# dune-community/pylrbms

Hardware: AMD Instinct MI355X
Metric: offline project+estimate throughput (higher is better)
Workload: dtype f64; 1 GPU; BASELINE.json config 3: 2D multiscale diffusion, 32x32 subdomains, k_c=4 (n=384 DG DoFs, n_rt=208 RT0 DoFs per subdomain), Q=2, local basis dim 40; subdomains=1024, N=40, Q=2, parallelism=subdomain tiles x1

## Files before the change

include/lrbms_hip.h:

```cpp
#ifndef LRBMS_HIP_H
#define LRBMS_HIP_H

#include <stdint.h>

#ifdef __cplusplus
extern "C" {
#endif

#define LRBMS_OK 0
#define LRBMS_E_INVALID (-1)
#define LRBMS_E_HIP (-2)
#define LRBMS_E_STATE (-3)
#define LRBMS_E_NOT_CONVERGED (-4)

#define LRBMS_NS 16

typedef struct lrbms_ctx lrbms_ctx;

typedef struct {
  int32_t kx, ky, n_T, n_rt, n_vertices, ncf;
  double hx, hy;
  double kappa[4];
  const int32_t* nb_elem;
  const int32_t* nb_face;
// ... 95 lines not shown
void* lrbms_ctx_aux_stream(lrbms_ctx* ctx, int32_t i);

#define LRBMS_OPT_OSWALD_VERTEX_PATCH 9
#define LRBMS_OPT_OSWALD_ZERO_ON_SUBDOMAIN_BOUNDARY 1
#define LRBMS_OPT_ACCUMULATE_COUPLING_ACROSS_Q 2
#define LRBMS_OPT_STREAMS 3
#define LRBMS_OPT_F1_KSPLIT 4
#define LRBMS_OPT_F1_FORM 5
#define LRBMS_OPT_COARSE 6
#define LRBMS_OPT_SOLVE_VALU 7
#define LRBMS_OPT_ESTIMATE_VALU 8
#define LRBMS_OPT_PREP_LDS 10
#define LRBMS_OPT_F2_FORM 11
#define LRBMS_OPT_SIDE_TABLES 12
#define LRBMS_OPT_THIN_MERGE 13
int lrbms_ctx_set_option(lrbms_ctx* ctx, int32_t option, int32_t value);

int lrbms_set_diagonal_neighbours(lrbms_ctx* ctx, const int32_t* nbr_diag);

int lrbms_fused_set_subset(lrbms_ctx* ctx, const int32_t* subset, int32_t count);

int lrbms_kernel_timing(lrbms_ctx* ctx, int32_t enable);
int lrbms_kernel_timing_read(lrbms_ctx* ctx, char* names, int64_t names_cap, double* ms, int32_t cap, int32_t* count);

int lrbms_project_estimate_fused_phase(lrbms_ctx* ctx, int32_t phase, int32_t Q, int32_t N, const double* V, const double* F,
                                       const double* A_diag, const double* A_cpl, const double* P_diag, const double* b,
                                       const double* ebar, const double* caa, const double* Aab, const double* Bbb, double* work,
                                       double* B_sys, double* rhs_red, double* E_red, double* M_red, double* G_nc, double* r_fd,
                                       double* G_rdd, double* G_bb, double* G_ab, double* G_aa, void* stream);

// ... 132 lines not shown
```

pylrbms_amd/_isa_check.py:

```python
import re


class IsaCheckError(RuntimeError):
    pass


def _functions(path):
    cur, out = None, {}
    with open(path) as fh:
        for ln in fh:
            m = re.match(r'^(_Z\w+):\s+; @', ln)
            if m:
                cur = m.group(1)
                out[cur] = []
                continue
            if cur is not None:
                if ln.startswith('.Lfunc_end'):
                    cur = None
                    continue
                out[cur].append(ln.rstrip('\n'))
    return out


def _metadata(path):
# ... 9 lines not shown
                continue
            m = re.match(r'^\s+(?:- )?\.(private_segment_fixed_size|sgpr_spill_count|vgpr_spill_count|vgpr_count|agpr_count):\s+(\d+)', ln)
            if m:
                key, val = m.group(1), int(m.group(2))
                if cur is not None and key not in out[cur]:
                    out[cur][key] = val
                else:
                    pending[key] = val
            if re.match(r'^\s+- \.', ln) and cur is not None and '.name' not in ln:
                cur = None
                m2 = re.match(r'^\s+- \.(\w+):\s+(\d+)', ln)
                pending = {m2.group(1): int(m2.group(2))} if m2 else {}
    return out


def _producer_loops(lines):
    in_asm, tags = False, []
    for ln in lines:
        s = ln.strip()
        if s.startswith(';;#ASMSTART'):
            in_asm = True
        tags.append(in_asm)
        if s.startswith(';;#ASMEND'):
            in_asm = False
    starts = [i for i, ln in enumerate(lines) if re.match(r'^(\.LBB\d+_\d+:|; %bb\.\d+:)', ln)]
    starts.append(len(lines))
    loops = {}
    for k in range(len(starts) - 1):
        head = lines[starts[k]]
        m = re.match(r'^\.LBB\d+_(\d+):.*Loop Header', head)
        owner = m.group(1) if m else None
        if owner is None:
            m = re.search(r'in Loop: Header=BB\d+_(\d+)', head)
            owner = m.group(1) if m else None
        if owner is not None:
            loops.setdefault(owner, []).extend(range(starts[k], starts[k + 1]))
    out = [idx for idx in loops.values() if any(tags[i] and 'global_load' in lines[i] for i in idx)]
    return out, tags


def _regs(tok):
    m = re.fullmatch(r'v(\d+)', tok)
    if m:
        return {int(m.group(1))}
    m = re.fullmatch(r'v\[(\d+):(\d+)\]', tok)
    if m:
        return set(range(int(m.group(1)), int(m.group(2)) + 1))
    return set()


def _operands(line):
    body = line.split(';')[0].strip()
# ... 120 lines not shown
        raise IsaCheckError('thin-kernel register check failed:\n  ' + '\n  '.join(problems))
    return sorted(report)


def check_fused_isa(asm_path):
    fns = _functions(asm_path)
    meta = _metadata(asm_path)
    report, problems = [], []
    with open(asm_path) as fh:
        try:
            report += check_thin_registers(fh.read())
        except IsaCheckError as exc:
            problems.append(str(exc))
    seen = 0
    for name, lines in fns.items():
        m = re.search(r'\dk_f(1u|1v|1|2g|2)I((?:Li\d+E)+)E', name) or re.search(r'\dk_f(1w)()E4Tmpl', name)
        if not m:
            continue
        kernel = 'k_f{}<{}>'.format(m.group(1), ','.join(re.findall(r'Li(\d+)E', m.group(2))))
        md = meta.get(name, {})
        spills = md.get('vgpr_spill_count', 0)
        scratch_lines = [i for i, ln in enumerate(lines) if re.match(r'\s+scratch_', ln)]
        in_asm = False
        first_asm_load = None
        for i, ln in enumerate(lines):
            st = ln.strip()
            if st.startswith(';;#ASMSTART'):
                in_asm = True
            elif st.startswith(';;#ASMEND'):
                in_asm = False
            elif in_asm and 'global_load' in ln:
                first_asm_load = i
                break
        wide = m.group(1) in ('1', '1u') and re.findall(r'Li(\d+)E', m.group(2))[0] == '4'
        if (spills or scratch_lines or md.get('private_segment_fixed_size', 0)) and not wide:
            problems.append('{}: scratch {} bytes, {} spilled VGPRs'.format(kernel, md.get('private_segment_fixed_size'), spills))
        if spills > 8:
            problems.append('{}: {} spilled VGPRs'.format(kernel, spills))
        if scratch_lines and first_asm_load is not None and max(scratch_lines) >= first_asm_load:
            problems.append('{}: scratch instruction behind the first asm-managed load (line {} >= {})'.format(
                kernel, max(scratch_lines), first_asm_load))
        lean = m.group(1) in ('1v', '1w')
        uses_asm_prefetch = any(';;#ASMSTART' in ln for ln in lines) and \
            any('global_load' in ln for ln in lines if True) and \
            any(re.search(r'^\s+s_waitcnt vmcnt\((?!0\))\d+\)\s*$' if not lean else r'^\s+s_waitcnt vmcnt\(0\)\s*$', ln) for ln in lines)
        loops, tags = _producer_loops(lines)
        if m.group(1) == '1' and kernel.endswith(',0>'):
            report.append('{}: compiler-managed loads, VGPRs {}'.format(kernel, md.get('vgpr_count')))
            continue
        if not loops or not uses_asm_prefetch:
            problems.append('{}: no producer loop with asm-managed prefetch found'.format(kernel))
            continue
        seen += 1
        if lean:
            loop_blocks = set()
            starts_all = sorted({0} | {i for i, ln in enumerate(lines) if re.match(r'^\.LBB\d+_\d+:', ln)})
            for idx in loops:
                members = set(idx)
                loop_blocks |= {b for b in starts_all if b in members}
            hz = _inflight_register_hazards(lines, tags, region=None, prologue_of=loop_blocks)
            if hz:
                problems.append('{}: compiler-emitted instruction touches the destination of an asm load of the PROLOGUE still in flight: {}'.format(
                    kernel, hz[:3]))
        for idx in loops:
            hazards = _inflight_register_hazards(lines, tags, region=idx)
            if hazards:
                problems.append('{}: compiler-emitted instruction touches the destination of an asm load still in flight: {}'.format(
                    kernel, hazards[:3]))
            a, b = idx[0], idx[-1]
            asm_waits = sorted({lines[k].strip() for k in idx if tags[k] and 'vmcnt' in lines[k]})
            counts = [int(x) for w in asm_waits for x in re.findall(r'vmcnt\((\d+)\)', w)]
            own_waits = [lines[k].strip() for k in idx if not tags[k] and re.search(r's_waitcnt.*vmcnt', lines[k])]
            own_vmem = [lines[k].strip() for k in idx
                        if not tags[k] and re.match(r'\s+(global_|buffer_|scratch_|flat_)', lines[k])]
            if not counts or (min(counts) == 0 and not lean):
                problems.append('{}: producer loop waits {} (expected one vmcnt(n), n > 0)'.format(kernel, asm_waits))
            if lean and counts and max(counts) != 0:
                problems.append('{}: staging loop waits {} (expected vmcnt(0) only)'.format(kernel, asm_waits))
# ... 36 lines not shown
```

pylrbms_amd/_native.py:

```python
import ctypes
import os

import numpy as np

_HERE = os.path.dirname(os.path.abspath(__file__))
LIB_PATH = os.path.join(_HERE, 'liblrbms_hip.so')

c_i32, c_i64, c_dbl, c_vp = ctypes.c_int32, ctypes.c_int64, ctypes.c_double, ctypes.c_void_p
_P_I32 = ctypes.POINTER(c_i32)
_P_DBL = ctypes.POINTER(c_dbl)


class MeshDesc(ctypes.Structure):
    _fields_ = ([(k, c_i32) for k in ('kx', 'ky', 'n_T', 'n_rt', 'n_vertices', 'ncf')] +
                [('hx', c_dbl), ('hy', c_dbl), ('kappa', c_dbl * 4)] +
                [(k, _P_I32) for k in ('nb_elem', 'nb_face', 'nb_elem_out', 'nb_face_out', 'elem_side_pos', 'elem_rt',
                                       'face_sign', 'dof_vertex', 'vdof_ptr', 'vdof_idx', 'rt_e0', 'rt_f0', 'rt_e1',
                                       'rt_f1', 'rt_side', 'side_elem', 'side_elem_out', 'side_count')] +
                [('ntouch', c_i32), ('touch_elem', _P_I32), ('touch_count', _P_I32)] +
                [(k, _P_DBL) for k in ('grad', 'area', 'normal', 'face_len', 'points')])


SIGNATURES = {
    'lrbms_version': (ctypes.c_char_p, []),
# ... 223 lines not shown
        self._check(self._fn('kernel_timing_read')(self.handle, names, 64 * cap, ms, cap, ctypes.byref(count)),
                    self.PREFIX + 'kernel_timing_read')
        nm = names.value.decode().split('\n') if count.value else []
        return [(nm[i], ms[i]) for i in range(count.value)]


class NativeContext(ContextBase):

    PREFIX = 'lrbms_'
    TIMING_CAP = 256
    _load = staticmethod(load_library)
    OPTIONS = {'oswald_zero_on_subdomain_boundary': 1, 'accumulate_coupling_across_q': 2, 'oswald_vertex_patch': 9, 'prep_lds': 10,
               'streams': 3, 'f1_ksplit': 4, 'f1_form': 5, 'coarse': 6, 'solve_valu': 7, 'estimate_valu': 8,
               'f2_form': 11,
               'side_tables': 12,
               'thin_merge': 13}
    S = S_ext = None
    _keep = None

    def mesh_upload(self, template, kappa, nbr, S, S_ext):
        t = template
        self.t, self.S, self.S_ext = t, int(S), int(S_ext)
        self.n_T, self.n, self.n_rt, self.ncf = t.n_T, t.n, t.n_rt, t.ncf
        self.nvs = max(t.nvx, t.nvy)
        arrs = {}
        d = MeshDesc()
        d.kx, d.ky, d.n_T, d.n_rt, d.n_vertices, d.ncf = t.kx, t.ky, t.n_T, t.n_rt, t.n_vertices, t.ncf
        d.hx, d.hy = t.hx, t.hy
        d.ntouch = t.ntouch
        kap = np.asarray(kappa, dtype=np.float64).reshape(4)
# ... 732 lines not shown
```

pylrbms_amd/csrc/capi.hip:

```cpp
#include <cmath>
#include <cstring>
#include <map>
#include <mutex>

#include "lrbms_dev.h"
#include "lrbms_pod.h"

int64_t estimator_work_size(lrbms_ctx* ctx, int Q, int N);
int64_t reduced_solve_work_size(lrbms_ctx* ctx, int N);
int launch_reduced_estimate_batch(lrbms_ctx* ctx, int Q, int N, int nmu, const double* theta, const double* u, const double* G_nc,
                                  const double* r_fd, const double* G_rdd, const double* G_bb, const double* G_ab,
                                  const double* G_aa, const double* Fside, const double* Fnc, const double* f2, const double* ceps,
                                  double hdiam, double* eta_loc, hipStream_t st);
int64_t reduced_solve_batch_work_size(lrbms_ctx* ctx, int N, int nmu);
int launch_reduced_solve_batch(lrbms_ctx* ctx, int Q, int N, int nmu, const double* theta, const double* B_sys,
                               const double* rhs_red, double* work, double* u, double rtol, int max_iter, double* info,
                               hipStream_t st);
int launch_assemble_dcorr(lrbms_ctx* ctx, int Q, const double* lam, double* D_corr, hipStream_t st);
int64_t local_correction_work_size(lrbms_ctx* ctx, int nmark);
int launch_local_correction(lrbms_ctx* ctx, int Q, const double* theta, int nmark, const int32_t* marked, const double* A_diag,
                            const double* A_cpl, const double* D_corr, const double* b, double* work, double* corr, double rtol,
                            int max_iter, double* info, hipStream_t st);
int64_t fom_solve_work_size(lrbms_ctx* ctx);
int launch_fom_solve(lrbms_ctx* ctx, int Q, const double* theta, const double* A_diag, const double* A_cpl, const double* b,
// ... 189 lines not shown
}

void* lrbms_ctx_aux_stream(lrbms_ctx* ctx, int32_t i) { return (ctx && i >= 0 && i < 3) ? (void*)ctx->aux[i] : nullptr; }

const char* lrbms_last_error(lrbms_ctx* ctx) { return ctx ? ctx->err.c_str() : "null context"; }

int lrbms_ctx_set_option(lrbms_ctx* ctx, int32_t option, int32_t value) {
  if (!ctx) return LRBMS_E_INVALID;
  int lo = 0, hi = 1;
  if (option == LRBMS_OPT_STREAMS) lo = -1;
  if (option == LRBMS_OPT_F1_KSPLIT) hi = 4;
  if (option == LRBMS_OPT_COARSE) hi = 2;
  if (option == LRBMS_OPT_PREP_LDS) hi = 3;
  if (option == LRBMS_OPT_F1_FORM) hi = 3;
  if (option == LRBMS_OPT_F2_FORM) hi = 2;
  if (value < lo || value > hi || (option == LRBMS_OPT_F1_KSPLIT && value == 3))
    return lrbms_fail(ctx, LRBMS_E_INVALID, "set_option: value out of range for this option");
  switch (option) {
    case LRBMS_OPT_OSWALD_ZERO_ON_SUBDOMAIN_BOUNDARY: ctx->t.opt_oswald_subdomain = value; break;
    case LRBMS_OPT_ACCUMULATE_COUPLING_ACROSS_Q: ctx->t.opt_accumulate_coupling = value; break;
    case LRBMS_OPT_OSWALD_VERTEX_PATCH:
      if (ctx->pass_ran && ctx->t.opt_oswald_vertex != value)
        return lrbms_fail(ctx, LRBMS_E_STATE, "set_option: LRBMS_OPT_OSWALD_VERTEX_PATCH cannot change after a fused pass has run on this context");
      ctx->t.opt_oswald_vertex = value;
      break;
    case LRBMS_OPT_STREAMS: ctx->opt_streams = value; break;
    case LRBMS_OPT_F1_KSPLIT: ctx->opt_f1_ksplit = value; break;
    case LRBMS_OPT_F1_FORM: ctx->opt_f1_legacy = value; break;
    case LRBMS_OPT_F2_FORM: ctx->opt_f2_form = value; break;
    case LRBMS_OPT_COARSE: ctx->opt_coarse = value; break;
    case LRBMS_OPT_SOLVE_VALU: ctx->opt_solve_valu = value; break;
    case LRBMS_OPT_ESTIMATE_VALU: ctx->opt_estimate_valu = value; break;
    case LRBMS_OPT_PREP_LDS: ctx->opt_prep_lds = value; break;
    case LRBMS_OPT_SIDE_TABLES: ctx->opt_side_tables = value; break;
    case LRBMS_OPT_THIN_MERGE: ctx->opt_thin_merge = value; break;
    default: return lrbms_fail(ctx, LRBMS_E_INVALID, "set_option: unknown option");
  }
  return LRBMS_OK;
}

int lrbms_set_diagonal_neighbours(lrbms_ctx* ctx, const int32_t* nbr_diag) {
  LRBMS_REQUIRE_MESH(ctx);
  if (!nbr_diag) return lrbms_fail(ctx, LRBMS_E_INVALID, "set_diagonal_neighbours: null table");
  for (long i = 0; i < (long)ctx->S * 4; ++i)
// ... 658 lines not shown
```

pylrbms_amd/csrc/fused.hip:

```cpp
#include <cstdlib>
#include <map>
#include <mutex>
#include <type_traits>
#include <utility>

#include "lrbms_dev.h"

namespace {

typedef double d4 __attribute__((ext_vector_type(4)));
typedef double d2 __attribute__((ext_vector_type(2)));
template <int W> struct VecT { using T = double; };
template <> struct VecT<2> { using T = d2; };
template <int W> __device__ inline typename VecT<W>::T ldv(const double* p) { return *reinterpret_cast<const typename VecT<W>::T*>(p); }
template <int W> __device__ inline typename VecT<W>::T ldv_off(const double* base, unsigned byte_off) {
  return *reinterpret_cast<const typename VecT<W>::T*>(reinterpret_cast<const char*>(base) + byte_off);
}
template <int W> __device__ inline void stv(double* p, typename VecT<W>::T v) { *reinterpret_cast<typename VecT<W>::T*>(p) = v; }
template <int W> __device__ inline typename VecT<W>::T zerov() { return typename VecT<W>::T(0.0); }
using W1 = std::integral_constant<int, 1>;
using W2 = std::integral_constant<int, 2>;

#if !defined(LRBMS_EXPERIMENT_BUILD) &&                                                                               \
    (defined(F1_NO_STAGE) || defined(F1_NO_APPLY) || defined(F1_NO_VALU_STAGE) || defined(F1_NO_MFMA) ||             \
// ... 2102 lines not shown
    return n;
  }
  static constexpr int slots(int role, int v) { return slots_before(role, v, count(role)); }
  static constexpr int max_slots(int role) { return slots(role, 0) > slots(role, 1) ? slots(role, 0) : slots(role, 1); }
  static constexpr bool tail_slot(int role, int v, int i) {
    for (int jt = 0; jt < count(role); ++jt)
      if (cls(first(role) + jt, v) == 3 && i == slots_before(role, v, jt) + 2) return true;
    return false;
  }
};
static_assert(F1wPlan::LDY % 32 == 16, "row stride of Ys");
static_assert(F1wPlan::cls(0, 0) < 3 && F1wPlan::cls(0, 1) < 3 && F1wPlan::cls(1, 0) < 3 && F1wPlan::cls(1, 1) < 3, "class-3 tiles are role B's");
template <int V> struct F1wV { static constexpr int value = V; };
constexpr int F1W_CSE = 4;

template <int ROLE>
__device__ __forceinline__ void f1w_body(const Tmpl& t, const F1Args& a, const double* __restrict__ Wab, double* __restrict__ Xs,
                                         double* __restrict__ Zs, double* __restrict__ Ys, double* __restrict__ Cs, double* __restrict__ red,
                                         int* __restrict__ flag, const int* __restrict__ colmap, const Grp* grp) {
  using LV = F1wPlan;
  constexpr int NTX = 3, QP = 2;
  constexpr int LDX = padded_ld(NTX);
  constexpr int LDY = LV::LDY;
  constexpr int NT = LV::count(ROLE), LV0 = LV::first(ROLE);
  constexpr int NS = LV::max_slots(ROLE);
  static_assert(NS <= F1V_SLOTS, "K-split partial layout");
  constexpr int NP = QP * (QP + 1) / 2;
  constexpr int NPAIR = NTX / 2, NSING = NTX % 2;
  const int s = subdomain_of(t, blockIdx.x), tid = threadIdx.x, lane = tid & 63, li = lane & 15, lk = lane >> 4;
  const int wave = uniform(tid >> 6), e = wave & 3;
  const int N = a.N, S = a.S, QN = QP * N;
  const int ksplit = gridDim.z;
  const int nchunks = t.nT / EC / ksplit;
  const int T0 = blockIdx.z * nchunks * EC;
  auto pos = [&](int g, int c) { return grp[g].cb[c >> 4] + (c & 15); };
  auto colc = [&](int ct) {
    return ct < 2 * NPAIR ? (32 * (ct >> 1) + 2 * li + 1 < N ? 32 * (ct >> 1) + 2 * li : N - 2) + (ct & 1) : (16 * ct + li < N ? 16 * ct + li : N - 1);
  };
  const double* Vs = (const double*)(((unsigned long long)__builtin_amdgcn_readfirstlane((int)((unsigned long long)(a.V + (long)s * t.n * N) >> 32)) << 32) |
                                     (unsigned)__builtin_amdgcn_readfirstlane((int)(unsigned long long)(a.V + (long)s * t.n * N)));

  d4 acc[NS];
#pragma unroll
  for (int i = 0; i < NS; ++i) acc[i] = (d4){0.0, 0.0, 0.0, 0.0};

  auto row_tile = [](d4& c, int i, double a16, const double (&at)[2], double bv) {
    if (i < 2) {
      c = __builtin_amdgcn_mfma_f64_16x16x4f64(a16, bv, c, 0, 0, 0);
    } else {
      c[0] = __builtin_amdgcn_mfma_f64_4x4x4f64(at[0], bv, c[0], 0, 0, 0);
      c[1] = __builtin_amdgcn_mfma_f64_4x4x4f64(at[1], bv, c[1], 0, 0, 0);
    }
  };
  constexpr int NSC = ROLE == 1 ? 3 : 1;
  int zc[NSC], cso[NSC];
  if constexpr (ROLE == 1) {
#pragma unroll
    for (int jt = 0; jt < NSC; ++jt) {
      const int m = colmap[(4 * (LV0 + jt) + e) * 16 + li];
// ... 43 lines not shown
              bv[jt] = Cb[(kk >> 1) * F1W_CSE + cso[jt % NSC]] * Zb[(kk + lk) * LDX + zc[jt % NSC]];
            else
              bv[jt] = Yb[(kk + lk) * LDY + (4 * (LV0 + jt) - LV::ytile_shift(LV0 + jt) + e) * 16 + li];
          }
        }
#pragma unroll
        for (int jt = 0; jt < NT; ++jt) {
          if (LV::kr(LV0 + jt, V) == 2) {
#pragma unroll
            for (int i = 0; i < LV::cls(LV0 + jt, V); ++i) row_tile(acc[LV::slots_before(ROLE, V, jt) + i], i, av[i], at, bv[jt]);
          }
        }
      }
    }
  };
  auto tie = [](double& v) { asm volatile("" : "+v"(v)); };
  auto tie2 = [](d2& v) { asm volatile("" : "+v"(v)); };
  double rhs_part[NTX];
#pragma unroll
  for (int ct = 0; ct < NTX; ++ct) rhs_part[ct] = 0.0;
  constexpr int R_GRP = 3 * (QP + 2);
  constexpr int R_B = R_GRP + 2, RRZ = R_GRP / 4, KQB = R_B % 4;
  static_assert(R_GRP % 4 == 0 && R_B / 4 == RRZ && R_B < 16, "the Z rows and b . V in one accumulator register");

  if constexpr (ROLE == 0) {
    struct Set {
      double A[3];
      d2 Bp[3][NPAIR];
      double Bs[3];
    };
    const int r16 = li, kq = lk;
    const double* ap[3];
    unsigned ainc = 0;
    int bbk[3];
    unsigned lcp[3][NPAIR], lcs[3];
#pragma unroll
    for (int ks = 0; ks < 3; ++ks) {
      const int k = 4 * ks + kq, bb = k / 3, cc = k - 3 * bb;
      bbk[ks] = bb;
      const double* src = t.zero64;
      unsigned stride = r16 < R_GRP ? 9 : r16 < R_B ? 6 : r16 == R_B ? 3 : 0;
      if (r16 < 3 * (QP + 1)) {
        const int g = r16 / 3, i = r16 % 3;
        src = (g < QP ? a.A_diag + ((long)g * S + s) * t.nT * 36 : a.P_diag + (long)s * t.nT * 36) + bb * 9 + i * 3 + cc;
        stride = 36;
      } else if (bb == 0 && r16 < R_GRP) {
        src = t.mass9 + (r16 - 3 * (QP + 1)) * 3 + cc;
      } else if (bb == 0 && r16 < R_B) {
        src = t.lgz + (r16 - R_GRP) * 3 + cc;
      } else if (bb == 0 && r16 == R_B) {
        src = a.b + (long)s * t.n + cc;
      }
      ap[ks] = src + (long)(T0 + e) * stride;
      ainc = 8u * EC * stride;
#pragma unroll
      for (int pp = 0; pp < NPAIR; ++pp) {
        const int col = 32 * pp + 2 * li + 1 < N ? 32 * pp + 2 * li : N - 2;
        lcp[ks][pp] = 8u * (unsigned)(cc * N + col);
      }
      const int cs = 16 * (NTX - 1) + li < N ? 16 * (NTX - 1) + li : N - 1;
      lcs[ks] = 8u * (unsigned)(cc * N + cs);
    }
    const unsigned rs3 = 24u * (unsigned)N;
    int xoff[NTX], zoff[NTX], yoff[3][NTX];
    const bool zrow = kq < 2;
#pragma unroll
    for (int ct = 0; ct < NTX; ++ct) {
      const int col = colc(ct);
      xoff[ct] = (3 * e + (kq < 3 ? kq : 0)) * LDX + col;
// ... 85 lines not shown
        for (int ct = 0; ct < NTX; ++ct) Zb[zoff[ct]] = D[ct][RRZ];
      }
      if (lane < NP) Cb[lane] = lane == 0 ? cc[0] : lane == 1 ? cc[1] : cc[2];
#pragma unroll
      for (int ct = 0; ct < NTX; ++ct) rhs_part[ct] += D[ct][RRZ];
      if (e == 0) F1_STAMP(0, c, 2);
      if (more) {
#pragma unroll
        for (int ks = 0; ks < 3; ++ks) ap[ks] = (const double*)((const char*)ap[ks] + ainc);
        load_set(T + EC, sc_nxt, cur);
      }
      if (e == 0) F1_STAMP(0, c, 3);
    };
    Set s0;
    Sc c0, c1;
    load_sc(T0 + e, c0);
    load_sc(nchunks > 1 ? T0 + EC + e : T0 + e, c1);
    load_set(T0 + e, c0, s0);
    auto round = [&](int c, Sc& x0, const Sc& x1) {
      stage(c, s0, x0, x1);
      lds_barrier();
      if (e == 0) F1_STAMP(0, c, 4);
      mfma_phase(c, F1wV<0>{});
      if (e == 0) F1_STAMP(0, c, 5);
    };
    for (int c = 0; c < nchunks; c += 2) {
      round(c, c0, c1);
      round(c + 1, c1, c0);
    }
    asm volatile("s_waitcnt vmcnt(0)" ::: "memory");
    tie_set(s0);
    if (a.rhs_red != nullptr && kq == KQB) {
#pragma unroll
      for (int ct = 0; ct < NTX; ++ct) {
        const int nat = ct < 2 * NPAIR ? 32 * (ct >> 1) + 2 * li + (ct & 1) : 16 * ct + li;
        if (nat < N) red[e * 64 + nat] = rhs_part[ct];
      }
    }
  } else {
    constexpr int NCI = 5, NPB = NCI / 2;
    struct Set {
      double A;
      d2 Bp[NPB];
      double Bs;
    };
    const double* Rs = (const double*)(((unsigned long long)__builtin_amdgcn_readfirstlane((int)((unsigned long long)(a.Rself + (long)s * t.nrt * QN) >> 32)) << 32) |
                                       (unsigned)__builtin_amdgcn_readfirstlane((int)(unsigned long long)(a.Rself + (long)s * t.nrt * QN)));
    const int kq = lk;
    const double* ap = t.zero64;
    if (kq < 3) ap = Wab + ((long)((li & 3) >> 1) * S + s) * t.nT * 6 + (li & 1) * 3 + kq;
    ap += (long)(T0 + e) * 6;
    unsigned lcp[NPB], lcs;
    int yo[NCI];
    {
      int col[NCI];
#pragma unroll
      for (int pp = 0; pp < NPB; ++pp) {
        col[2 * pp] = 32 * pp + 2 * li + 1 < QN ? 32 * pp + 2 * li : QN - 2;
        col[2 * pp + 1] = col[2 * pp] + 1;
        lcp[pp] = 8u * (unsigned)col[2 * pp];
      }
      col[NCI - 1] = 32 * NPB + li < QN ? 32 * NPB + li : QN - 1;
      lcs = 8u * (unsigned)col[NCI - 1];
#pragma unroll
      for (int m = 0; m < NCI; ++m) {
        const int q2 = col[m] >= N ? 1 : 0;
// ... 37 lines not shown
      double D[NCI];
#pragma unroll
      for (int m = 0; m < NCI; ++m) D[m] = __builtin_amdgcn_mfma_f64_4x4x4f64(cur.A, bop(cur, m), 0.0, 0, 0, 0);
#pragma unroll
      for (int m = 0; m < NCI; ++m) Yb[yo[m]] = D[m];
      if (e == 0) F1_STAMP(1, c, 2);
      if (more) {
        ap += 6 * EC;
        load_set(sc_nxt, cur);
      }
      if (e == 0) F1_STAMP(1, c, 3);
    };
    auto run = [&](auto vtag) {
      Set s0;
      Sc c0, c1;
      load_sc(T0 + e, c0);
      load_set(c0, s0);
      load_sc(nchunks > 1 ? T0 + EC + e : T0 + e, c0);
      auto round = [&](int c, const Sc& x0, Sc& x1) {
        stage(c, s0, x0, x1);
        lds_barrier();
        if (e == 0) F1_STAMP(1, c, 4);
        mfma_phase(c, vtag);
        if (e == 0) F1_STAMP(1, c, 5);
      };
      for (int c = 0; c < nchunks; c += 2) {
        round(c, c0, c1);
        round(c + 1, c1, c0);
      }
      asm volatile("s_waitcnt vmcnt(0)" ::: "memory");
      tie_set(s0);
    };
    if (e < 2) run(F1wV<0>{});
    else run(F1wV<1>{});
  }
  if (ksplit > 1) {
    constexpr int PW = F1V_SLOTS * 4 * 64;
    const long wg = 8L * PW + 64;
    double* mine = a.part + ((long)s * ksplit + blockIdx.z) * wg;
    double* pw = mine + (long)wave * PW + 2 * lane;
    auto put = [&](auto vtag) {
      constexpr int V = decltype(vtag)::value;
#pragma unroll
      for (int i = 0; i < NS; ++i)
#pragma unroll
        for (int h = 0; h < (LV::tail_slot(ROLE, V, i) ? 1 : 2); ++h) store_sc1_b128(pw + (i * 2 + h) * 128, acc[i][2 * h], acc[i][2 * h + 1]);
// ... 21 lines not shown
        const double* pz = all + z * wg + (long)wave * PW + 2 * lane;
#pragma unroll
        for (int i = 0; i < NS; ++i)
#pragma unroll
          for (int r = 0; r < (LV::tail_slot(ROLE, V, i) ? 2 : 4); ++r) acc[i][r] += load_sc1_b64(pz + (i * 2 + r / 2) * 128 + r % 2);
      }
    };
    if (ROLE == 0 || e < 2) gather(F1wV<0>{});
    else gather(F1wV<1>{});
    if (a.rhs_red != nullptr && tid < N) {
      double sum = 0.0;
      for (int z = 0; z < ksplit; ++z) sum += load_sc1_b64(all + z * wg + 8L * PW + tid);
      a.rhs_red[(long)s * N + tid] = sum;
    }
  }
  auto epilogue = [&](auto vtag) {
    constexpr int V = decltype(vtag)::value;
#pragma unroll
    for (int jt = 0; jt < NT; ++jt) {
      const int m = colmap[(4 * (LV0 + jt) + e) * 16 + li];
      const bool live = m >= 0;
      const int g = live ? m >> 8 : 0, jj = m & 255;
      const int ld = grp[g].ld;
      const bool sym = grp[g].sym != 0;
      double* base = grp[g].dst + (long)s * grp[g].sstride;
      double* base_t = grp[g].dst_t ? grp[g].dst_t + (long)s * grp[g].sstride : nullptr;
#pragma unroll
      for (int i = 0; i < LV::cls(LV0 + jt, V); ++i) {
#pragma unroll
        for (int r = 0; r < (i < 2 ? 4 : 2); ++r) {
          const int row = i * 16 + lk + 4 * r;
          const double val = acc[LV::slots_before(ROLE, V, jt) + i][r];
          if (live && row < N && (!sym || row <= jj)) {
            base[(long)row * ld + jj] = val;
            if (sym && row < jj) base[(long)jj * ld + row] = val;
            if (base_t) base_t[(long)jj * ld + row] = val;
          }
        }
      }
    }
  };
  if (ROLE == 0 || e < 2) epilogue(F1wV<0>{});
  else epilogue(F1wV<1>{});
}

__global__ __launch_bounds__(512, 2) void k_f1w(Tmpl t, F1Args a, GrpTable gt, const double* __restrict__ Wab) {
  constexpr int NTX = 3, NTYS = F1wPlan::NL;
  constexpr int LDX = padded_ld(NTX);
  constexpr int LDY = F1wPlan::LDY;
  __shared__ double Xs[2 * 3 * EC * LDX];
  __shared__ double Zs[2 * 2 * EC * LDX];
  __shared__ double Ys[2 * 3 * EC * LDY];
  __shared__ double Cs[2 * EC * F1W_CSE];
  __shared__ double red[EC * 64];
  __shared__ int colmap[4 * NTYS * 16];
  __shared__ Grp grp[F1_MAXG];
  __shared__ int flag;
  const int tid = threadIdx.x;
#pragma unroll
  for (int g = 0; g < F1_MAXG; ++g)
    if (tid == g) grp[g] = gt.g[g];
  for (int i = tid; i < 2 * 3 * EC * LDX; i += 512) Xs[i] = 0.0;
  for (int i = tid; i < 2 * 2 * EC * LDX; i += 512) Zs[i] = 0.0;
  for (int i = tid; i < 2 * 3 * EC * LDY; i += 512) Ys[i] = 0.0;
  for (int i = tid; i < 4 * NTYS * 16; i += 512) colmap[i] = -1;
  if (tid < EC * 64) red[tid] = 0.0;
  __syncthreads();
  for (int i = tid; i < gt.n * a.N; i += 512) {
    const int g = i / a.N, c = i - g * a.N;
    colmap[grp[g].cb[c >> 4] + (c & 15)] = (g << 8) | c;
  }
  __syncthreads();
  if (uniform(tid >> 6) < EC)
    f1w_body<0>(t, a, Wab, Xs, Zs, Ys, Cs, red, &flag, colmap, grp);
  else
    f1w_body<1>(t, a, Wab, Xs, Zs, Ys, Cs, red, &flag, colmap, grp);
  if (gridDim.z == 1 && a.rhs_red != nullptr) {
    __syncthreads();
    if (tid < a.N) {
      double sum = 0.0;
      for (int w = 0; w < EC; ++w) sum += red[w * 64 + tid];
      a.rhs_red[(long)subdomain_of(t, blockIdx.x) * a.N + tid] = sum;
    }
  }
}

__global__ __launch_bounds__(256) void k_f1_zero(GrpTable gt, int S, int N, double* __restrict__ rhs_red, const int* __restrict__ sub_list) {
  const int s = sub_list ? sub_list[blockIdx.x] : blockIdx.x;
  for (int g = 0; g < gt.n; ++g) {
    double* dst = gt.g[g].dst + (long)s * gt.g[g].sstride;
    double* dst_t = gt.g[g].dst_t ? gt.g[g].dst_t + (long)s * gt.g[g].sstride : nullptr;
    const int ld = gt.g[g].ld;
    for (int i = threadIdx.x; i < N * N; i += 256) {
      dst[(long)(i / N) * ld + i % N] = 0.0;
      if (dst_t) dst_t[(long)(i / N) * ld + i % N] = 0.0;
    }
  }
// ... 1996 lines not shown
          ctx->ksp_ticket = nullptr;
          ctx->ksp_ticket_cap = 0;
          LRBMS_HIP_CHECK(ctx, hipMalloc(&ctx->ksp_ticket, sizeof(int) * (size_t)S));
          LRBMS_HIP_CHECK(ctx, hipMemset(ctx->ksp_ticket, 0, sizeof(int) * (size_t)S));
          ctx->ksp_ticket_cap = S;
        }
        a.part = ctx->ksp_part;
        a.ticket = ctx->ksp_ticket;
      }
      if (ksplit > 1 && !unified) {
        for (int sl = 0; sl < nsl; ++sl)
          hipLaunchKernelGGL(k_f1_zero, dim3(Sg), dim3(256), 0, st, gt[sl], S, N, sl == 0 ? a.rhs_red : nullptr, t.sub_list);
      }
      const dim3 grid(Sg, nsl, ksplit);
      KScope ks(ctx, lean2 ? "k_f1w" : lean ? "k_f1v" : unified ? "k_f1u" : "k_f1", st);
      if (lean2) {
        hipLaunchKernelGGL(k_f1w, grid, dim3(512), 0, st, t, a, gt[0], Wab);
        LRBMS_LAUNCH_CHECK(ctx);
        continue;
      }
      if (lean) {
#define LRBMS_F1V(A, B, C, D, E)                                               \
  if (ntx == A && Q == B && lv[0] == C && lv[1] == D && lv[2] == E)            \
    hipLaunchKernelGGL((k_f1v<A, B, C, D, E>), grid, dim3(512), 0, st, t, a, gt[0]);
        LRBMS_F1V_LIST(LRBMS_F1V)
#undef LRBMS_F1V
        LRBMS_LAUNCH_CHECK(ctx);
        continue;
      }
      const size_t ldsf1u = sizeof(double) * 9 * (t.nT / ksplit);
// ... 219 lines not shown
```

pylrbms_amd/csrc/lrbms_dev.h:

```cpp
#pragma once
#include <hip/hip_runtime.h>
#include <stdint.h>
#include <string>
#include <vector>

#include "lrbms_ctx_base.h"

struct Tmpl {
  int kx, ky, nT, n, nrt, nv, nvx, nvy, ncf;
  double hx, hy;
  double kappa[4], kinv[4], kmin;
  const int *nb_elem, *nb_face, *nb_elem_out, *nb_face_out, *elem_side_pos, *elem_rt, *face_sign;
  const int *dof_vertex, *vdof_ptr, *vdof_idx;
  const int *rt_e0, *rt_f0, *rt_e1, *rt_f1, *rt_side;
  const int *side_elem, *side_elem_out, *side_count;
  int ntouch;
  const int *touch_elem, *touch_count;
  const double *grad, *area, *normal, *face_len, *points;
  const double* stiff;
  const double* mass9;
  const double* zero64;
  const double* lgz;
  const double* hab;
  const int* touch_vtx;
// ... 42 lines not shown
  long asm_counter = 0;
  const double* asm_ptr[SRC_COUNT] = {nullptr, nullptr, nullptr, nullptr};
  int asm_Q = 0;
  double* stab = nullptr;
  long stab_cap = 0;
  const double* stab_ptr[SRC_COUNT] = {nullptr, nullptr, nullptr, nullptr};
  long stab_gen[SRC_COUNT] = {0, 0, 0, 0};
  int stab_Q = 0;
  int opt_side_tables = 1;
  int opt_thin_merge = 1;
  bool pass_ran = false;
  bool diag_explicit = false;
  int* subset = nullptr;
  int subset_n = 0, subset_cap = 0;
  lrbms_quadrature* qdev = nullptr;
  int opt_streams = -1, opt_f1_ksplit = 0, opt_f1_legacy = 0, opt_coarse = 1, opt_solve_valu = 0, opt_estimate_valu = 0, opt_prep_lds = 1, opt_f2_form = 0;
  double* src_phi = nullptr;
  const double* user_pc = nullptr;
  int user_pc_N = 0;
};

#define SIGMA_INNER 8.0
#define SIGMA_BOUNDARY 14.0

__host__ __device__ inline int side_to_slot(int side) { return side < 2 ? side : side + 1; }
__host__ __device__ inline int slot_to_side(int slot) { return slot < 2 ? slot : slot - 1; }

int build_template_tables(lrbms_ctx* ctx);
int launch_wab(lrbms_ctx* ctx, int Q, const double* Aab, double* Wab, hipStream_t st);
inline void note_assembled(lrbms_ctx* ctx, int kind, const double* p) {
  std::vector<lrbms_ctx::AsmRec>& known = ctx->asm_known[kind];
// ... 58 lines not shown
```

Before: 1.760 million subdomains/s.

## Add persistent-workgroup variant of the f1w projection kernel with cross-item prefetch

Adds k_f1wp, a persistent kernel that launches about one workgroup per CU and loops over subdomains. Each workgroup issues the next subdomain's prologue loads while it writes the previous subdomain's epilogue, and it double-buffers the rhs reduction. The aim is to remove per-block launch and ramp-up cost and to hide tail latency between subdomains. By default it is used when ksplit is 1 and there are more subdomains than CUs. The cost is more complex pointer-rebasing logic and an ISA checker extended to validate the nested item loop.

New measurement: 1.777 million subdomains/s (median of 6 runs). Within noise of the previous version (+1.0%).

```diff
diff --git a/include/lrbms_hip.h b/include/lrbms_hip.h
--- a/include/lrbms_hip.h
+++ b/include/lrbms_hip.h
@@ -133,6 +133,7 @@
 #define LRBMS_OPT_F2_FORM 11
 #define LRBMS_OPT_SIDE_TABLES 12
 #define LRBMS_OPT_THIN_MERGE 13
+#define LRBMS_OPT_F1_WGS 14
 int lrbms_ctx_set_option(lrbms_ctx* ctx, int32_t option, int32_t value);
 
 int lrbms_set_diagonal_neighbours(lrbms_ctx* ctx, const int32_t* nbr_diag);
diff --git a/pylrbms_amd/_isa_check.py b/pylrbms_amd/_isa_check.py
--- a/pylrbms_amd/_isa_check.py
+++ b/pylrbms_amd/_isa_check.py
@@ -47,7 +47,7 @@
     return out
 
 
-def _producer_loops(lines):
+def _producer_loops(lines, item_loops=None):
     in_asm, tags = False, []
     for ln in lines:
         s = ln.strip()
@@ -58,17 +58,32 @@
             in_asm = False
     starts = [i for i, ln in enumerate(lines) if re.match(r'^(\.LBB\d+_\d+:|; %bb\.\d+:)', ln)]
     starts.append(len(lines))
-    loops = {}
+    loops, outer, parent = {}, set(), {}
     for k in range(len(starts) - 1):
         head = lines[starts[k]]
-        m = re.match(r'^\.LBB\d+_(\d+):.*Loop Header', head)
-        owner = m.group(1) if m else None
+        m = re.match(r'^\.LBB\d+_(\d+):', head)
+        note = head
+        for ln in lines[starts[k] + 1:starts[k + 1]]:
+            if not re.match(r'^\s+;', ln):
+                break
+            note += ln
+        owner = m.group(1) if m and 'Loop Header' in note else None
+        if owner is not None and 'Inner Loop Header' not in note:
+            outer.add(owner)
+        mp = re.search(r'Parent Loop BB\d+_(\d+)', note)
+        if owner is not None and mp:
+            parent[owner] = mp.group(1)
         if owner is None:
             m = re.search(r'in Loop: Header=BB\d+_(\d+)', head)
             owner = m.group(1) if m else None
         if owner is not None:
             loops.setdefault(owner, []).extend(range(starts[k], starts[k + 1]))
-    out = [idx for idx in loops.values() if any(tags[i] and 'global_load' in lines[i] for i in idx)]
+    if item_loops is None:
+        outer = set()
+    out = [idx for o, idx in loops.items() if o not in outer and any(tags[i] and 'global_load' in lines[i] for i in idx)]
+    if item_loops is not None:
+        item_loops.extend((idx, sorted(idx + [i for c, ci in loops.items() if parent.get(c) == o for i in ci]))
+                          for o, idx in loops.items() if o in outer)
     return out, tags
 
 
@@ -219,7 +234,7 @@
             problems.append(str(exc))
     seen = 0
     for name, lines in fns.items():
-        m = re.search(r'\dk_f(1u|1v|1|2g|2)I((?:Li\d+E)+)E', name) or re.search(r'\dk_f(1w)()E4Tmpl', name)
+        m = re.search(r'\dk_f(1u|1v|1|2g|2)I((?:Li\d+E)+)E', name) or re.search(r'\dk_f(1wp?)()E4Tmpl', name)
         if not m:
             continue
         kernel = 'k_f{}<{}>'.format(m.group(1), ','.join(re.findall(r'Li(\d+)E', m.group(2))))
@@ -245,11 +260,12 @@
         if scratch_lines and first_asm_load is not None and max(scratch_lines) >= first_asm_load:
             problems.append('{}: scratch instruction behind the first asm-managed load (line {} >= {})'.format(
                 kernel, max(scratch_lines), first_asm_load))
-        lean = m.group(1) in ('1v', '1w')
+        lean = m.group(1) in ('1v', '1w', '1wp')
         uses_asm_prefetch = any(';;#ASMSTART' in ln for ln in lines) and \
             any('global_load' in ln for ln in lines if True) and \
             any(re.search(r'^\s+s_waitcnt vmcnt\((?!0\))\d+\)\s*$' if not lean else r'^\s+s_waitcnt vmcnt\(0\)\s*$', ln) for ln in lines)
-        loops, tags = _producer_loops(lines)
+        nest = [] if m.group(1) == '1wp' else None
+        loops, tags = _producer_loops(lines, nest)
         if m.group(1) == '1' and kernel.endswith(',0>'):
             report.append('{}: compiler-managed loads, VGPRs {}'.format(kernel, md.get('vgpr_count')))
             continue
@@ -260,13 +276,33 @@
         if lean:
             loop_blocks = set()
             starts_all = sorted({0} | {i for i, ln in enumerate(lines) if re.match(r'^\.LBB\d+_\d+:', ln)})
-            for idx in loops:
+            for idx in loops + [whole for _, whole in nest or []]:
                 members = set(idx)
                 loop_blocks |= {b for b in starts_all if b in members}
             hz = _inflight_register_hazards(lines, tags, region=None, prologue_of=loop_blocks)
             if hz:
                 problems.append('{}: compiler-emitted instruction touches the destination of an asm load of the PROLOGUE still in flight: {}'.format(
                     kernel, hz[:3]))
+        if nest is not None:
+            if len(nest) < len(loops):
+                problems.append('{}: {} staging loops, {} item loops around them'.format(kernel, len(loops), len(nest)))
+            for idx, whole in nest:
+                hz = _inflight_register_hazards(lines, tags, region=whole)
+                if hz:
+                    problems.append('{}: compiler-emitted instruction touches the destination of an asm load still in flight (item loop): {}'.format(
+                        kernel, hz[:3]))
+                own_waits = [lines[k].strip() for k in idx if not tags[k] and re.search(r's_waitcnt.*vmcnt', lines[k])]
+                own_loads = [lines[k].strip() for k in idx
+                             if not tags[k] and re.match(r'\s+((global|buffer|flat)_(load|atomic)|scratch_)', lines[k])]
+                counts = [int(x) for k in idx if tags[k] for x in re.findall(r'vmcnt\((\d+)\)', lines[k])]
+                if own_waits:
+                    problems.append('{}: compiler-emitted vmcnt wait in the item loop: {}'.format(kernel, own_waits[:2]))
+                if own_loads:
+                    problems.append('{}: compiler-emitted vector load in the item loop: {}'.format(kernel, own_loads[:2]))
+                if counts and max(counts) != 0:
+                    problems.append('{}: item loop waits vmcnt({}) (expected vmcnt(0) only)'.format(kernel, max(counts)))
+                report.append('{}: item loop [{}..{}], {} compiler stores'.format(
+                    kernel, idx[0], idx[-1], sum(1 for k in idx if not tags[k] and re.match(r'\s+(global|flat)_store', lines[k]))))
         for idx in loops:
             hazards = _inflight_register_hazards(lines, tags, region=idx)
             if hazards:
diff --git a/pylrbms_amd/_native.py b/pylrbms_amd/_native.py
--- a/pylrbms_amd/_native.py
+++ b/pylrbms_amd/_native.py
@@ -261,6 +261,7 @@
                'streams': 3, 'f1_ksplit': 4, 'f1_form': 5, 'coarse': 6, 'solve_valu': 7, 'estimate_valu': 8,
                'f2_form': 11,
                'side_tables': 12,
+               'f1_wgs': 14,
                'thin_merge': 13}
     S = S_ext = None
     _keep = None
diff --git a/pylrbms_amd/csrc/capi.hip b/pylrbms_amd/csrc/capi.hip
--- a/pylrbms_amd/csrc/capi.hip
+++ b/pylrbms_amd/csrc/capi.hip
@@ -227,6 +227,7 @@
   if (option == LRBMS_OPT_PREP_LDS) hi = 3;
   if (option == LRBMS_OPT_F1_FORM) hi = 3;
   if (option == LRBMS_OPT_F2_FORM) hi = 2;
+  if (option == LRBMS_OPT_F1_WGS) hi = 1 << 20;
   if (value < lo || value > hi || (option == LRBMS_OPT_F1_KSPLIT && value == 3))
     return lrbms_fail(ctx, LRBMS_E_INVALID, "set_option: value out of range for this option");
   switch (option) {
@@ -241,6 +242,7 @@
     case LRBMS_OPT_F1_KSPLIT: ctx->opt_f1_ksplit = value; break;
     case LRBMS_OPT_F1_FORM: ctx->opt_f1_legacy = value; break;
     case LRBMS_OPT_F2_FORM: ctx->opt_f2_form = value; break;
+    case LRBMS_OPT_F1_WGS: ctx->opt_f1_wgs = value; break;
     case LRBMS_OPT_COARSE: ctx->opt_coarse = value; break;
     case LRBMS_OPT_SOLVE_VALU: ctx->opt_solve_valu = value; break;
     case LRBMS_OPT_ESTIMATE_VALU: ctx->opt_estimate_valu = value; break;
diff --git a/pylrbms_amd/csrc/fused.hip b/pylrbms_amd/csrc/fused.hip
--- a/pylrbms_amd/csrc/fused.hip
+++ b/pylrbms_amd/csrc/fused.hip
@@ -2140,10 +2140,10 @@
 template <int V> struct F1wV { static constexpr int value = V; };
 constexpr int F1W_CSE = 4;
 
-template <int ROLE>
+template <int ROLE, bool PERSIST = false>
 __device__ __forceinline__ void f1w_body(const Tmpl& t, const F1Args& a, const double* __restrict__ Wab, double* __restrict__ Xs,
                                          double* __restrict__ Zs, double* __restrict__ Ys, double* __restrict__ Cs, double* __restrict__ red,
-                                         int* __restrict__ flag, const int* __restrict__ colmap, const Grp* grp) {
+                                         int* __restrict__ flag, const int* __restrict__ colmap, const Grp* grp, int items = 0) {
   using LV = F1wPlan;
   constexpr int NTX = 3, QP = 2;
   constexpr int LDX = padded_ld(NTX);
@@ -2153,22 +2153,32 @@
   static_assert(NS <= F1V_SLOTS, "K-split partial layout");
   constexpr int NP = QP * (QP + 1) / 2;
   constexpr int NPAIR = NTX / 2, NSING = NTX % 2;
-  const int s = subdomain_of(t, blockIdx.x), tid = threadIdx.x, lane = tid & 63, li = lane & 15, lk = lane >> 4;
+  int item = blockIdx.x;
+  int s = subdomain_of(t, item);
+  const int tid = threadIdx.x, lane = tid & 63, li = lane & 15, lk = lane >> 4;
   const int wave = uniform(tid >> 6), e = wave & 3;
   const int N = a.N, S = a.S, QN = QP * N;
-  const int ksplit = gridDim.z;
+  const int ksplit = PERSIST ? 1 : gridDim.z;
   const int nchunks = t.nT / EC / ksplit;
-  const int T0 = blockIdx.z * nchunks * EC;
+  const int T0 = PERSIST ? 0 : blockIdx.z * nchunks * EC;
+  if (e == 0) F1_STAMP(ROLE, 1, 6);
   auto pos = [&](int g, int c) { return grp[g].cb[c >> 4] + (c & 15); };
   auto colc = [&](int ct) {
     return ct < 2 * NPAIR ? (32 * (ct >> 1) + 2 * li + 1 < N ? 32 * (ct >> 1) + 2 * li : N - 2) + (ct & 1) : (16 * ct + li < N ? 16 * ct + li : N - 1);
   };
-  const double* Vs = (const double*)(((unsigned long long)__builtin_amdgcn_readfirstlane((int)((unsigned long long)(a.V + (long)s * t.n * N) >> 32)) << 32) |
-                                     (unsigned)__builtin_amdgcn_readfirstlane((int)(unsigned long long)(a.V + (long)s * t.n * N)));
+  auto sbase = [](const double* p) {
+    return (const double*)(((unsigned long long)__builtin_amdgcn_readfirstlane((int)((unsigned long long)p >> 32)) << 32) |
+                           (unsigned)__builtin_amdgcn_readfirstlane((int)(unsigned long long)p));
+  };
+  auto next_sub = [&](int it) { return t.sub_list ? ((cint_p)t.sub_list)[uniform(it)] : uniform(it); };
+  const double* Vs = sbase(a.V + (long)s * t.n * N);
 
   d4 acc[NS];
-#pragma unroll
-  for (int i = 0; i < NS; ++i) acc[i] = (d4){0.0, 0.0, 0.0, 0.0};
+  auto zero_acc = [&] {
+#pragma unroll
+    for (int i = 0; i < NS; ++i) acc[i] = (d4){0.0, 0.0, 0.0, 0.0};
+  };
+  zero_acc();
 
   auto row_tile = [](d4& c, int i, double a16, const double (&at)[2], double bv) {
     if (i < 2) {
@@ -2242,6 +2252,32 @@
       }
     }
   };
+  auto epilogue = [&](auto vtag, int sd) {
+    constexpr int V = decltype(vtag)::value;
+#pragma unroll
+    for (int jt = 0; jt < NT; ++jt) {
+      const int m = colmap[(4 * (LV0 + jt) + e) * 16 + li];
+      const bool live = m >= 0;
+      const int g = live ? m >> 8 : 0, jj = m & 255;
+      const int ld = grp[g].ld;
+      const bool sym = grp[g].sym != 0;
+      double* base = grp[g].dst + (long)sd * grp[g].sstride;
+      double* base_t = grp[g].dst_t ? grp[g].dst_t + (long)sd * grp[g].sstride : nullptr;
+#pragma unroll
+      for (int i = 0; i < LV::cls(LV0 + jt, V); ++i) {
+#pragma unroll
+        for (int r = 0; r < (i < 2 ? 4 : 2); ++r) {
+          const int row = i * 16 + lk + 4 * r;
+          const double val = acc[LV::slots_before(ROLE, V, jt) + i][r];
+          if (live && row < N && (!sym || row <= jj)) {
+            base[(long)row * ld + jj] = val;
+            if (sym && row < jj) base[(long)jj * ld + row] = val;
+            if (base_t) base_t[(long)jj * ld + row] = val;
+          }
+        }
+      }
+    }
+  };
   auto tie = [](double& v) { asm volatile("" : "+v"(v)); };
   auto tie2 = [](d2& v) { asm volatile("" : "+v"(v)); };
   double rhs_part[NTX];
@@ -2262,10 +2298,8 @@
     unsigned ainc = 0;
     int bbk[3];
     unsigned lcp[3][NPAIR], lcs[3];
-#pragma unroll
-    for (int ks = 0; ks < 3; ++ks) {
+    auto item_ap = [&](int ks) {
       const int k = 4 * ks + kq, bb = k / 3, cc = k - 3 * bb;
-      bbk[ks] = bb;
       const double* src = t.zero64;
       unsigned stride = r16 < R_GRP ? 9 : r16 < R_B ? 6 : r16 == R_B ? 3 : 0;
       if (r16 < 3 * (QP + 1)) {
@@ -2281,6 +2315,12 @@
       }
       ap[ks] = src + (long)(T0 + e) * stride;
       ainc = 8u * EC * stride;
+    };
+#pragma unroll
+    for (int ks = 0; ks < 3; ++ks) {
+      const int k = 4 * ks + kq, bb = k / 3, cc = k - 3 * bb;
+      bbk[ks] = bb;
+      item_ap(ks);
 #pragma unroll
       for (int pp = 0; pp < NPAIR; ++pp) {
         const int col = 32 * pp + 2 * li + 1 < N ? 32 * pp + 2 * li : N - 2;
@@ -2396,9 +2436,11 @@
     };
     Set s0;
     Sc c0, c1;
-    load_sc(T0 + e, c0);
-    load_sc(nchunks > 1 ? T0 + EC + e : T0 + e, c1);
-    load_set(T0 + e, c0, s0);
+    auto prologue = [&] {
+      load_sc(T0 + e, c0);
+      load_sc(nchunks > 1 ? T0 + EC + e : T0 + e, c1);
+      load_set(T0 + e, c0, s0);
+    };
     auto round = [&](int c, Sc& x0, const Sc& x1) {
       stage(c, s0, x0, x1);
       lds_barrier();
@@ -2406,18 +2448,78 @@
       mfma_phase(c, F1wV<0>{});
       if (e == 0) F1_STAMP(0, c, 5);
     };
-    for (int c = 0; c < nchunks; c += 2) {
-      round(c, c0, c1);
-      round(c + 1, c1, c0);
-    }
-    asm volatile("s_waitcnt vmcnt(0)" ::: "memory");
-    tie_set(s0);
-    if (a.rhs_red != nullptr && kq == KQB) {
-#pragma unroll
-      for (int ct = 0; ct < NTX; ++ct) {
-        const int nat = ct < 2 * NPAIR ? 32 * (ct >> 1) + 2 * li + (ct & 1) : 16 * ct + li;
-        if (nat < N) red[e * 64 + nat] = rhs_part[ct];
-      }
+    auto deposit = [&](double* rd) {
+      if (a.rhs_red != nullptr && kq == KQB) {
+#pragma unroll
+        for (int ct = 0; ct < NTX; ++ct) {
+          const int nat = ct < 2 * NPAIR ? 32 * (ct >> 1) + 2 * li + (ct & 1) : 16 * ct + li;
+          if (nat < N) rd[e * 64 + nat] = rhs_part[ct];
+        }
+      }
+    };
+    if constexpr (!PERSIST) {
+      prologue();
+      for (int c = 0; c < nchunks; c += 2) {
+        round(c, c0, c1);
+        round(c + 1, c1, c0);
+      }
+      if (e == 0) F1_STAMP(0, 2, 6);
+      asm volatile("s_waitcnt vmcnt(0)" ::: "memory");
+      tie_set(s0);
+      deposit(red);
+    } else {
+      const int G = gridDim.x;
+      int s_pend = -1, par = 0;
+      int s_done = -1;
+      prologue();
+      for (;;) {
+        stage(0, s0, c0, c1);
+        if (s_done >= 0) {
+          epilogue(F1wV<0>{}, s_done);
+          zero_acc();
+        }
+        lds_barrier();
+        if (e == 0) F1_STAMP(0, 0, 4);
+        mfma_phase(0, F1wV<0>{});
+        if (e == 0) F1_STAMP(0, 0, 5);
+        round(1, c1, c0);
+        for (int c = 2; c < nchunks; c += 2) {
+          round(c, c0, c1);
+          round(c + 1, c1, c0);
+        }
+        if (e == 0) F1_STAMP(0, 2, 6);
+        asm volatile("s_waitcnt vmcnt(0)" ::: "memory");
+        tie_set(s0);
+        if (a.rhs_red != nullptr) {
+          if (wave == 0 && s_pend >= 0 && lane < N) {
+            const double* rd = red + (par ^ 1) * EC * 64;
+            double sum = 0.0;
+            for (int w = 0; w < EC; ++w) sum += rd[w * 64 + lane];
+            a.rhs_red[(long)s_pend * N + lane] = sum;
+          }
+          deposit(red + par * EC * 64);
+#pragma unroll
+          for (int ct = 0; ct < NTX; ++ct) rhs_part[ct] = 0.0;
+          s_pend = s;
+          par ^= 1;
+        }
+        if (item + G >= items) break;
+        const int s_old = s;
+        s_done = s;
+        item += G;
+        s = next_sub(item);
+        Vs = sbase(a.V + (long)s * t.n * N);
+#pragma unroll
+        for (int ks = 0; ks < 3; ++ks) {
+          const long sst = r16 < 3 * (QP + 1) ? (long)t.nT * 36 : (4 * ks + kq < 3 && r16 == R_B) ? (long)t.n : 0L;
+          ap[ks] = (const double*)((const char*)ap[ks] - (long)(nchunks - 1) * ainc) + (long)(s - s_old) * sst;
+        }
+        load_sc(T0 + e, c0);
+        load_sc(nchunks > 1 ? T0 + EC + e : T0 + e, c1);
+        touch_sc(c0);
+        load_set(T0 + e, c0, s0);
+      }
+      epilogue(F1wV<0>{}, s);
     }
   } else {
     constexpr int NCI = 5, NPB = NCI / 2;
@@ -2426,12 +2528,15 @@
       d2 Bp[NPB];
       double Bs;
     };
-    const double* Rs = (const double*)(((unsigned long long)__builtin_amdgcn_readfirstlane((int)((unsigned long long)(a.Rself + (long)s * t.nrt * QN) >> 32)) << 32) |
-                                       (unsigned)__builtin_amdgcn_readfirstlane((int)(unsigned long long)(a.Rself + (long)s * t.nrt * QN)));
+    const double* Rs = sbase(a.Rself + (long)s * t.nrt * QN);
     const int kq = lk;
-    const double* ap = t.zero64;
-    if (kq < 3) ap = Wab + ((long)((li & 3) >> 1) * S + s) * t.nT * 6 + (li & 1) * 3 + kq;
-    ap += (long)(T0 + e) * 6;
+    const double* ap;
+    auto item_ap = [&] {
+      ap = t.zero64;
+      if (kq < 3) ap = Wab + ((long)((li & 3) >> 1) * S + s) * t.nT * 6 + (li & 1) * 3 + kq;
+      ap += (long)(T0 + e) * 6;
+    };
+    item_ap();
     unsigned lcp[NPB], lcs;
     int yo[NCI];
     {
@@ -2499,9 +2604,11 @@
     auto run = [&](auto vtag) {
       Set s0;
       Sc c0, c1;
-      load_sc(T0 + e, c0);
-      load_set(c0, s0);
-      load_sc(nchunks > 1 ? T0 + EC + e : T0 + e, c0);
+      auto prologue = [&] {
+        load_sc(T0 + e, c0);
+        load_set(c0, s0);
+        load_sc(nchunks > 1 ? T0 + EC + e : T0 + e, c0);
+      };
       auto round = [&](int c, const Sc& x0, Sc& x1) {
         stage(c, s0, x0, x1);
         lds_barrier();
@@ -2509,12 +2616,52 @@
         mfma_phase(c, vtag);
         if (e == 0) F1_STAMP(1, c, 5);
       };
-      for (int c = 0; c < nchunks; c += 2) {
-        round(c, c0, c1);
-        round(c + 1, c1, c0);
-      }
-      asm volatile("s_waitcnt vmcnt(0)" ::: "memory");
-      tie_set(s0);
+      if constexpr (!PERSIST) {
+        prologue();
+        for (int c = 0; c < nchunks; c += 2) {
+          round(c, c0, c1);
+          round(c + 1, c1, c0);
+        }
+        if (e == 0) F1_STAMP(1, 2, 6);
+        asm volatile("s_waitcnt vmcnt(0)" ::: "memory");
+        tie_set(s0);
+      } else {
+        const int G = gridDim.x;
+        int s_done = -1;
+        prologue();
+        for (;;) {
+          stage(0, s0, c0, c1);
+          if (s_done >= 0) {
+            epilogue(vtag, s_done);
+            zero_acc();
+          }
+          lds_barrier();
+          if (e == 0) F1_STAMP(1, 0, 4);
+          mfma_phase(0, vtag);
+          if (e == 0) F1_STAMP(1, 0, 5);
+          round(1, c1, c0);
+          for (int c = 2; c < nchunks; c += 2) {
+            round(c, c0, c1);
+            round(c + 1, c1, c0);
+          }
+          if (e == 0) F1_STAMP(1, 2, 6);
+          asm volatile("s_waitcnt vmcnt(0)" ::: "memory");
+          tie_set(s0);
+          if (item + G >= items) break;
+          const int s_old = s;
+          s_done = s;
+          item += G;
+          s = next_sub(item);
+          Rs = sbase(a.Rself + (long)s * t.nrt * QN);
+          ap += (long)(s - s_old) * (kq < 3 ? (long)t.nT * 6 : 0L) - (long)(nchunks - 1) * 6 * EC;
+          load_sc(T0 + e, c0);
+#pragma unroll
+          for (int f = 0; f < 3; ++f) asm volatile("" ::"s"(c0.rt[f]) : "memory");
+          load_set(c0, s0);
+          load_sc(nchunks > 1 ? T0 + EC + e : T0 + e, c0);
+        }
+        epilogue(vtag, s);
+      }
     };
     if (e < 2) run(F1wV<0>{});
     else run(F1wV<1>{});
@@ -2566,34 +2713,15 @@
       a.rhs_red[(long)s * N + tid] = sum;
     }
   }
-  auto epilogue = [&](auto vtag) {
-    constexpr int V = decltype(vtag)::value;
-#pragma unroll
-    for (int jt = 0; jt < NT; ++jt) {
-      const int m = colmap[(4 * (LV0 + jt) + e) * 16 + li];
-      const bool live = m >= 0;
-      const int g = live ? m >> 8 : 0, jj = m & 255;
-      const int ld = grp[g].ld;
-      const bool sym = grp[g].sym != 0;
-      double* base = grp[g].dst + (long)s * grp[g].sstride;
-      double* base_t = grp[g].dst_t ? grp[g].dst_t + (long)s * grp[g].sstride : nullptr;
-#pragma unroll
-      for (int i = 0; i < LV::cls(LV0 + jt, V); ++i) {
-#pragma unroll
-        for (int r = 0; r < (i < 2 ? 4 : 2); ++r) {
-          const int row = i * 16 + lk + 4 * r;
-          const double val = acc[LV::slots_before(ROLE, V, jt) + i][r];
-          if (live && row < N && (!sym || row <= jj)) {
-            base[(long)row * ld + jj] = val;
-            if (sym && row < jj) base[(long)jj * ld + row] = val;
-            if (base_t) base_t[(long)jj * ld + row] = val;
-          }
-        }
-      }
-    }
-  };
-  if (ROLE == 0 || e < 2) epilogue(F1wV<0>{});
-  else epilogue(F1wV<1>{});
+  if constexpr (!PERSIST) {
+    if (ROLE == 0 || e < 2) epilogue(F1wV<0>{}, s);
+    else epilogue(F1wV<1>{}, s);
+  }
+  if (e == 0) F1_STAMP(ROLE, 3, 6);
+#ifdef F1_TRACE
+  asm volatile("s_waitcnt vmcnt(0)" ::: "memory");
+#endif
+  if (e == 0) F1_STAMP(ROLE, 4, 6);
 }
 
 __global__ __launch_bounds__(512, 2) void k_f1w(Tmpl t, F1Args a, GrpTable gt, const double* __restrict__ Wab) {
@@ -2609,6 +2737,7 @@
   __shared__ Grp grp[F1_MAXG];
   __shared__ int flag;
   const int tid = threadIdx.x;
+  if (((tid >> 6) & 3) == 0) F1_STAMP((tid >> 8) & 1, 0, 6);
 #pragma unroll
   for (int g = 0; g < F1_MAXG; ++g)
     if (tid == g) grp[g] = gt.g[g];
@@ -2633,6 +2762,49 @@
       double sum = 0.0;
       for (int w = 0; w < EC; ++w) sum += red[w * 64 + tid];
       a.rhs_red[(long)subdomain_of(t, blockIdx.x) * a.N + tid] = sum;
+    }
+  }
+}
+
+__global__ __launch_bounds__(512, 2) void k_f1wp(Tmpl t, F1Args a, GrpTable gt, const double* __restrict__ Wab, int items) {
+  constexpr int NTX = 3, NTYS = F1wPlan::NL;
+  constexpr int LDX = padded_ld(NTX);
+  constexpr int LDY = F1wPlan::LDY;
+  __shared__ double Xs[2 * 3 * EC * LDX];
+  __shared__ double Zs[2 * 2 * EC * LDX];
+  __shared__ double Ys[2 * 3 * EC * LDY];
+  __shared__ double Cs[2 * EC * F1W_CSE];
+  __shared__ double red[2 * EC * 64];
+  __shared__ int colmap[4 * NTYS * 16];
+  __shared__ Grp grp[F1_MAXG];
+  const int tid = threadIdx.x;
+  if (((tid >> 6) & 3) == 0) F1_STAMP((tid >> 8) & 1, 0, 6);
+#pragma unroll
+  for (int g = 0; g < F1_MAXG; ++g)
+    if (tid == g) grp[g] = gt.g[g];
+  for (int i = tid; i < 2 * 3 * EC * LDX; i += 512) Xs[i] = 0.0;
+  for (int i = tid; i < 2 * 2 * EC * LDX; i += 512) Zs[i] = 0.0;
+  for (int i = tid; i < 2 * 3 * EC * LDY; i += 512) Ys[i] = 0.0;
+  for (int i = tid; i < 4 * NTYS * 16; i += 512) colmap[i] = -1;
+  if (tid < 2 * EC * 64) red[tid] = 0.0;
+  __syncthreads();
+  for (int i = tid; i < gt.n * a.N; i += 512) {
+    const int g = i / a.N, c = i - g * a.N;
+    colmap[grp[g].cb[c >> 4] + (c & 15)] = (g << 8) | c;
+  }
+  __syncthreads();
+  if (uniform(tid >> 6) < EC)
+    f1w_body<0, true>(t, a, Wab, Xs, Zs, Ys, Cs, red, nullptr, colmap, grp, items);
+  else
+    f1w_body<1, true>(t, a, Wab, Xs, Zs, Ys, Cs, red, nullptr, colmap, grp, items);
+  if (a.rhs_red != nullptr) {
+    const int mine = (items - (int)blockIdx.x + (int)gridDim.x - 1) / (int)gridDim.x;
+    __syncthreads();
+    if (tid < a.N) {
+      const double* rd = red + ((mine - 1) & 1) * EC * 64;
+      double sum = 0.0;
+      for (int w = 0; w < EC; ++w) sum += rd[w * 64 + tid];
+      a.rhs_red[(long)subdomain_of(t, (int)blockIdx.x + (mine - 1) * (int)gridDim.x) * a.N + tid] = sum;
     }
   }
 }
@@ -4659,6 +4831,19 @@
       }
       const dim3 grid(Sg, nsl, ksplit);
       KScope ks(ctx, lean2 ? "k_f1w" : lean ? "k_f1v" : unified ? "k_f1u" : "k_f1", st);
+      if (lean2 && ksplit == 1) {
+        if (ctx->num_cus == 0) {
+          int ncu = 0;
+          LRBMS_HIP_CHECK(ctx, hipDeviceGetAttribute(&ncu, hipDeviceAttributeMultiprocessorCount, ctx->device));
+          ctx->num_cus = ncu > 0 ? ncu : 256;
+        }
+        const int wgs = ctx->opt_f1_wgs > 0 ? std::min(ctx->opt_f1_wgs, Sg) : Sg > ctx->num_cus ? ctx->num_cus : 0;
+        if (wgs > 0) {
+          hipLaunchKernelGGL(k_f1wp, dim3(wgs), dim3(512), 0, st, t, a, gt[0], Wab, Sg);
+          LRBMS_LAUNCH_CHECK(ctx);
+          continue;
+        }
+      }
       if (lean2) {
         hipLaunchKernelGGL(k_f1w, grid, dim3(512), 0, st, t, a, gt[0], Wab);
         LRBMS_LAUNCH_CHECK(ctx);
diff --git a/pylrbms_amd/csrc/lrbms_dev.h b/pylrbms_amd/csrc/lrbms_dev.h
--- a/pylrbms_amd/csrc/lrbms_dev.h
+++ b/pylrbms_amd/csrc/lrbms_dev.h
@@ -80,7 +80,7 @@
   int* subset = nullptr;
   int subset_n = 0, subset_cap = 0;
   lrbms_quadrature* qdev = nullptr;
-  int opt_streams = -1, opt_f1_ksplit = 0, opt_f1_legacy = 0, opt_coarse = 1, opt_solve_valu = 0, opt_estimate_valu = 0, opt_prep_lds = 1, opt_f2_form = 0;
+  int opt_streams = -1, opt_f1_ksplit = 0, opt_f1_legacy = 0, opt_coarse = 1, opt_solve_valu = 0, opt_estimate_valu = 0, opt_prep_lds = 1, opt_f2_form = 0, opt_f1_wgs = 0;
   double* src_phi = nullptr;
   const double* user_pc = nullptr;
   int user_pc_N = 0;
```
